# irfanfadhullah/unet_zoo

Measured on AMD Instinct MI355X. Metric: images/sec (fwd+bwd) at B=16 3x256x256, 1/2/4/8 MI355X, higher is better.
Workload: dtype bf16; 1 GPU; unet train step (zero_grad+fwd+BCE+bwd+clip+AdamW), B=16/GPU 3x256x256, random-init weights; global_batch=16, parallelism=dp1

## Files before the change

### include/unetzoo_hip.h

```cpp
#ifndef UNETZOO_HIP_H
#define UNETZOO_HIP_H

#include <stddef.h>
#include <stdint.h>

#ifdef __cplusplus
extern "C" {
#endif

#define UZ_ABI_VERSION 1

enum { UZ_F32 = 0, UZ_BF16 = 1 };

enum {
  UZ_OK = 0,
  UZ_EINVAL = -1,
  UZ_ENOTIMPL = -2
};

enum {
  UZ_TAPS_CONV = 0,
  UZ_TAPS_GATHER2X2 = 1,
  UZ_TAPS_CONV_UP2 = 2,
  UZ_TAPS_CONV_S2 = 3
};
enum {
  UZ_STORE_PLAIN = 0,
  UZ_STORE_SHUFFLE2X2 = 1
};

int uz_abi_version(void);
const char* uz_last_error_string(void);
int uz_profile_arm(void* start_event, void* stop_event);
int uz_profile_disarm(void);
int uz_build_ablate(void);
const char* uz_source_hash(void);
int uz_clock_probe(int iters, void* out_pairs, int workgroups, void* stream);
int uz_set_cu_reserve(int n);
int uz_get_cu_reserve(void);

typedef struct uz_conv_desc {
  int dtype;
  int N, H, W;
  int Hin, Win;
  int Cin, ldx;
  int Nout, ldy;
  int ntaps, taps_mode, dil;
  int store_mode, Co;
  int Hout, Wout;
} uz_conv_desc;

int uz_conv_igemm_grid_m(const uz_conv_desc* d);
int uz_conv_igemm_kernel_name(const uz_conv_desc* d, int with_workspace, char* buf, int cap);
int uz_conv_igemm(const uz_conv_desc* d, const void* x, const void* w_packed, const float* bias,
                  void* y, float* stats_partial, void* stream);
int uz_conv_igemm_res(const uz_conv_desc* d, const void* x, const void* w_packed, const float* bias,
                      const void* res, int ldres, void* y, void* stream);
int uz_conv_igemm_res_ws(const uz_conv_desc* d, const void* x, const void* w_packed, const float* bias,
                         const void* res, int ldres, void* y, void* workspace, void* stream);
long long uz_conv_igemm_workspace_bytes(const uz_conv_desc* d);
int uz_conv_igemm_ws_grid_m(const uz_conv_desc* d);
int uz_conv_igemm_ws(const uz_conv_desc* d, const void* x, const void* w_packed, const float* bias,
                     void* y, float* stats_partial, void* workspace, void* stream);
int uz_conv_igemm_bnred_supported(const uz_conv_desc* d);
int uz_conv_igemm_bnred(const uz_conv_desc* d, const void* x, const void* w_packed, void* y, const void* bn_y,
                        int ld_bny, const float* scale, const float* shift, const float* mean, const float* invstd,
                        float* partial, void* stream);

int uz_conv_igemm_xf_supported(const uz_conv_desc* d);
int uz_conv_igemm_xf(const uz_conv_desc* d, const void* x, const float* in_scale, const float* in_shift,
                     const void* w_packed, const float* bias, void* y, float* stats_partial, void* stream);

int uz_conv_igemm_bnact_supported(const uz_conv_desc* d);
int uz_conv_igemm_bnact(const uz_conv_desc* d, const void* x, const void* w_packed, const float* bias,
                        const float* out_scale, const float* out_shift, int relu, void* y, void* stream);

typedef struct uz_wgrad_desc {
  int dtype;
  int N, H, W;
  int Hr, Wr;
  int Ci, ldl;
  int Cj, ldr;
  int ntaps, taps_mode, dil;
} uz_wgrad_desc;

int uz_wgrad_split(const uz_wgrad_desc* d);
long long uz_wgrad_workspace_bytes(const uz_wgrad_desc* d);
int uz_wgrad(const uz_wgrad_desc* d, const void* L, const void* R, float* out, void* workspace,
             void* stream);
int uz_wgrad_kernel_name(const uz_wgrad_desc* d, char* buf, int cap);
int uz_wgrad_xf_supported(const uz_wgrad_desc* d);
int uz_wgrad_xf(const uz_wgrad_desc* d, const void* L, const void* R, const float* r_scale, const float* r_shift,
// ... 416 lines not shown
```

### unet_zoo_amd/_lib.py

```python
from __future__ import annotations

import ctypes
import os
from ctypes import POINTER, Structure, c_char_p, c_double, c_float, c_int, c_void_p

import torch

UZ_F32, UZ_BF16 = 0, 1
TAPS_CONV, TAPS_GATHER2X2, TAPS_CONV_UP2, TAPS_CONV_S2 = 0, 1, 2, 3
STORE_PLAIN, STORE_SHUFFLE2X2 = 0, 1
PACK_CONV_FWD, PACK_CONV_DGRAD, PACK_CONVT_FWD, PACK_CONVT_DGRAD, PACK_IM2COL, PACK_VEC_REPEAT = range(6)

LIB_NAME = "libunetzoo_hip.so"
LIB_PATH = os.environ.get("UNET_ZOO_AMD_LIB") or os.path.join(os.path.dirname(os.path.abspath(__file__)), LIB_NAME)

EXPORTS = (
    "uz_abi_version", "uz_last_error_string", "uz_build_ablate", "uz_source_hash", "uz_set_cu_reserve", "uz_get_cu_reserve", "uz_clock_probe", "uz_conv_igemm_grid_m", "uz_conv_igemm",
    "uz_wgrad_split", "uz_wgrad_workspace_bytes", "uz_wgrad", "uz_wgrad_kernel_name", "uz_wgrad_phase", "uz_wgrad_xf_supported", "uz_wgrad_xf", "uz_conv3x3_first_supported", "uz_conv3x3_first_rows", "uz_conv3x3_first_fwd",
    "uz_conv3x3_first_wgrad_workspace_bytes", "uz_conv3x3_first_wgrad", "uz_conv3x3_first_wgrad_bn", "uz_pack_weights", "uz_pack_weights_batched", "uz_pack_conv3x3_batched", "uz_im2col3x3_nchw", "uz_bn_finalize",
    "uz_bn_eval_scale", "uz_bn_relu_apply", "uz_bn_relu_bwd_workspace_bytes", "uz_bn_relu_bwd_reduce", "uz_bn_relu_bwd_apply",
    "uz_outconv_fwd", "uz_outconv_fwd_xf", "uz_outconv_bwd_workspace_bytes", "uz_outconv_bwd", "uz_outconv_bwd_rows", "uz_outconv_bwd_bnred", "uz_bn_relu_bwd_apply_head_supported", "uz_bn_relu_bwd_apply_head",
    "uz_colsum",
    "uz_attn_grid", "uz_attn_psi_fwd", "uz_attn_gate_fwd", "uz_attn_bwd_psi", "uz_attn_bwd_reduce",
    "uz_attn_bwd_apply", "uz_sum_rows", "uz_sum_rows_f32", "uz_sum2x2",
    "uz_bn_relu_add_apply", "uz_bn_relu_add_apply_fin", "uz_bn_relu_bwd_reduce_rows", "uz_bn_relu_bwd_apply_fin", "uz_bilinear_fwd", "uz_bilinear_bwd", "uz_resize_bilinear_fwd", "uz_resize_bilinear_bwd", "uz_resample2",
    "uz_pool_grad_combine",
    "uz_sideconv3x3_fwd", "uz_sideconv3x3_bwd_workspace_bytes", "uz_sideconv3x3_bwd",
    "uz_fuse1x1_fwd", "uz_fuse1x1_bwd_workspace_bytes", "uz_fuse1x1_bwd",
    "uz_conv_igemm_workspace_bytes", "uz_conv_igemm_ws_grid_m", "uz_conv_igemm_ws",
    "uz_conv_igemm_bnred_supported", "uz_conv_igemm_bnred", "uz_conv_igemm_xf_supported", "uz_conv_igemm_xf", "uz_conv_igemm_kernel_name", "uz_bn_bwd_finalize", "uz_profile_arm", "uz_profile_disarm",
    "uz_patchify", "uz_layernorm_fwd", "uz_layernorm_bwd_rows", "uz_layernorm_bwd", "uz_layernorm_act_bwd",
    "uz_ln_head_fwd", "uz_ln_head_bwd_workspace_bytes", "uz_ln_head_bwd", "uz_sum_rows_f32_ld",
    "uz_winattn_fwd", "uz_winattn_bwd_rows", "uz_winattn_bwd",
    "uz_colsum_workspace_bytes", "uz_colsum_ws", "uz_colstats_rows", "uz_colstats", "uz_cpb_fwd", "uz_cpb_bwd",
    "uz_cpb_fwd_batched", "uz_cpb_bwd_batched_workspace_bytes", "uz_cpb_bwd_batched",
    "uz_clip_adamw_workspace_bytes", "uz_clip_adamw",
    "uz_gelu_fwd", "uz_gelu_bwd", "uz_dwconv3x3", "uz_dwconv3x3_wgrad_rows", "uz_dwconv3x3_wgrad",
    "uz_space_to_depth", "uz_space_to_depth_crop", "uz_im2col_nchw", "uz_sra_fwd", "uz_sra_bwd_workspace_bytes", "uz_sra_bwd",
    "uz_bce_dice_workspace_bytes", "uz_bce_dice", "uz_colsum_batched_workspace_bytes", "uz_colsum_batched", "uz_sum_rows_f32_batched", "uz_conv_igemm_res", "uz_wgrad_multi_workspace_bytes", "uz_wgrad_multi", "uz_conv_igemm_res_ws",
    "uz_add_relu", "uz_relu_bwd", "uz_pil_resample_h_u8", "uz_pil_resample_v_f32",
    "uz_gemm_nt", "uz_softmax_fwd", "uz_softmax_bwd", "uz_adaptive_avgpool_fwd", "uz_adaptive_avgpool_bwd",
    "uz_rowdot_f32", "uz_cast_rows", "uz_wgrad_batched_workspace_bytes", "uz_wgrad_batched", "uz_wgrad_batched2",
    "uz_softmax_workspace_bytes", "uz_add_map", "uz_dropout", "uz_chanscale_relu", "uz_chanattn_probs_fwd", "uz_chanattn_probs_bwd",
    "uz_conv5x5_grid_m", "uz_conv5x5", "uz_wgrad5x5_workspace_bytes", "uz_wgrad5x5",
    "uz_bn_elu_apply", "uz_bn_elu_bwd_rows", "uz_bn_elu_bwd_reduce", "uz_bn_elu_bwd_apply",
    "uz_conv_igemm_bnact_supported", "uz_conv_igemm_bnact", "uz_conv3x3_first_fwd_bnact",
    "uz_region_loss_workspace_bytes", "uz_region_loss",
    "uz_class_loss_workspace_bytes", "uz_class_loss",
)


class ConvDesc(Structure):
    _fields_ = [(n, c_int) for n in (
        "dtype", "N", "H", "W", "Hin", "Win", "Cin", "ldx", "Nout", "ldy", "ntaps", "taps_mode",
        "dil", "store_mode", "Co", "Hout", "Wout")]


class WgradDesc(Structure):
    _fields_ = [(n, c_int) for n in (
        "dtype", "N", "H", "W", "Hr", "Wr", "Ci", "ldl", "Cj", "ldr", "ntaps", "taps_mode", "dil")]


class Conv5Desc(Structure):
    _fields_ = [(n, c_int) for n in ("dtype", "N", "H", "W", "Cin", "ldx", "Nout", "ldy", "ksize")]


class Wgrad5Desc(Structure):
    _fields_ = [(n, c_int) for n in ("dtype", "N", "H", "W", "Ci", "ldl", "Cj", "ldr", "ksize", "CiOut", "CjOut")]


# ... 62 lines not shown
REGION_MAX_ITEMS = 64


class RegionItem(Structure):
    _fields_ = [("logits", c_void_p), ("target", c_void_p), ("dlogits", c_void_p), ("weight", c_float)]


class RegionDesc(Structure):
    _fields_ = [("n_items", c_int), ("n", ctypes.c_longlong), ("groups", c_int)] \
        + [(n, c_float) for n in ("w_bce", "w_region", "alpha", "beta", "smooth", "gamma", "pos_weight")] \
        + [("metric_item", c_int)]


CLASS_MAX_ITEMS = 16
CLASS_MAX_K = 32
CLASS_REDUCE_BATCH, CLASS_REDUCE_IMAGE = 0, 1


class ClassItem(Structure):
    _fields_ = [("logits", c_void_p), ("dlogits", c_void_p), ("weight", c_float)]


class ClassDesc(Structure):
    _fields_ = [("n_items", c_int), ("N", c_int), ("K", c_int), ("HW", ctypes.c_longlong)] \
        + [(n, c_float) for n in ("w_ce", "w_dice", "smooth", "label_smoothing")] \
        + [(n, c_int) for n in ("ignore_index", "reduce", "include_background", "square", "metric_item")]


class HipLibraryError(RuntimeError):
    pass


_lib = None


def load():
    global _lib
    if _lib is not None:
        return _lib
    if not os.path.exists(LIB_PATH):
        raise HipLibraryError(
            f"{LIB_PATH} not found: the HIP kernel library is not built. Run "
            "`python -c 'import __graft_entry__ as g; g.build()'` from the repo root. "
            "unet_zoo_amd has no CPU fallback.")
    lib = ctypes.CDLL(LIB_PATH)
    lib.uz_abi_version.restype = c_int
    lib.uz_last_error_string.restype = c_char_p
    lib.uz_source_hash.restype = c_char_p
    lib.uz_source_hash.argtypes = []
    vp, ip, fp = c_void_p, c_int, c_float
    lib.uz_set_cu_reserve.argtypes = [c_int]
    lib.uz_clock_probe.argtypes = [c_int, vp, c_int, vp]
    lib.uz_get_cu_reserve.argtypes = []
    lib.uz_conv_igemm_grid_m.argtypes = [POINTER(ConvDesc)]
    lib.uz_conv_igemm.argtypes = [POINTER(ConvDesc), vp, vp, vp, vp, vp, vp]
    lib.uz_conv_igemm_res.argtypes = [POINTER(ConvDesc), vp, vp, vp, vp, ip, vp, vp]
    lib.uz_conv_igemm_res_ws.argtypes = [POINTER(ConvDesc), vp, vp, vp, vp, ip, vp, vp, vp]
    lib.uz_conv_igemm_workspace_bytes.argtypes = [POINTER(ConvDesc)]
    lib.uz_conv_igemm_ws_grid_m.argtypes = [POINTER(ConvDesc)]
    lib.uz_conv_igemm_ws.argtypes = [POINTER(ConvDesc), vp, vp, vp, vp, vp, vp, vp]
    lib.uz_conv_igemm_bnred_supported.argtypes = [POINTER(ConvDesc)]
    lib.uz_conv_igemm_xf_supported.argtypes = [POINTER(ConvDesc)]
    lib.uz_conv_igemm_xf.argtypes = [POINTER(ConvDesc), vp, vp, vp, vp, vp, vp, vp, vp]
    lib.uz_conv_igemm_bnact_supported.argtypes = [POINTER(ConvDesc)]
    lib.uz_conv_igemm_bnact.argtypes = [POINTER(ConvDesc), vp, vp, vp, vp, vp, c_int, vp, vp]
    lib.uz_conv_igemm_kernel_name.argtypes = [POINTER(ConvDesc), c_int, c_char_p, c_int]
    lib.uz_profile_arm.argtypes = [vp, vp]
    lib.uz_profile_disarm.argtypes = []
    lib.uz_conv_igemm_bnred.argtypes = [POINTER(ConvDesc), vp, vp, vp, vp, c_int, vp, vp, vp, vp, vp, vp]
    lib.uz_bn_bwd_finalize.argtypes = [vp, c_int, c_int, vp, vp, vp, vp]
    lib.uz_patchify.argtypes = [ip, vp, ip, ip, ip, ip, ip, ip, vp, vp]
    lib.uz_layernorm_fwd.argtypes = [POINTER(LnDesc), vp, vp, vp, vp, vp, vp, vp, vp]
    lib.uz_layernorm_act_bwd.argtypes = [POINTER(LnDesc), vp, vp, vp, vp, vp, vp, vp, vp]
    lib.uz_layernorm_bwd_rows.argtypes = [POINTER(LnDesc)]
    lib.uz_layernorm_bwd.argtypes = [POINTER(LnDesc), vp, vp, vp, vp, vp, vp, vp, vp]
    lib.uz_ln_head_fwd.argtypes = [POINTER(LnDesc), vp, vp, vp, vp, vp, ip, vp, vp, vp]
    lib.uz_ln_head_bwd_workspace_bytes.argtypes = [POINTER(LnDesc), ip]
    lib.uz_ln_head_bwd.argtypes = [POINTER(LnDesc), vp, vp, vp, vp, ip, vp, vp, vp, vp, vp, vp, vp, vp, vp]
    lib.uz_sum_rows_f32_ld.argtypes = [vp, ip, ip, ip, vp, ip, vp, vp]
    lib.uz_winattn_fwd.argtypes = [POINTER(WinAttnDesc), vp, vp, vp, vp, vp, vp]
    lib.uz_winattn_bwd_rows.argtypes = [POINTER(WinAttnDesc)]
    lib.uz_winattn_bwd.argtypes = [POINTER(WinAttnDesc), vp, vp, vp, vp, vp, vp, ip, vp, ip, vp, vp]
    lib.uz_colstats_rows.argtypes = [ip, ip, ip]
    lib.uz_colstats.argtypes = [ip, vp, ip, ip, ip, vp, vp]
    lib.uz_cpb_fwd.argtypes = [vp, vp, vp, vp, vp, ip, ip, ip, vp, vp]
    lib.uz_cpb_bwd.argtypes = [vp, vp, vp, vp, vp, ip, ip, ip, vp, vp, vp, vp, vp]
    lib.uz_cpb_fwd_batched.argtypes = [vp, ip, vp]
    lib.uz_cpb_bwd_batched_workspace_bytes.argtypes = [vp, ip]
    lib.uz_cpb_bwd_batched.argtypes = [vp, ip, vp, vp]
    lib.uz_clip_adamw_workspace_bytes.argtypes = []
    lib.uz_clip_adamw.argtypes = [vp, vp, vp, vp, ctypes.c_longlong, fp, fp, fp, fp, fp, fp, vp, vp, vp]
    lib.uz_wgrad_split.argtypes = [POINTER(WgradDesc)]
    lib.uz_wgrad_workspace_bytes.argtypes = [POINTER(WgradDesc)]
    lib.uz_wgrad.argtypes = [POINTER(WgradDesc), vp, vp, vp, vp, vp]
    lib.uz_wgrad_kernel_name.argtypes = [POINTER(WgradDesc), c_char_p, c_int]
    lib.uz_wgrad_phase.argtypes = [POINTER(WgradDesc), vp, vp, vp, vp, vp, c_int]
    lib.uz_wgrad_xf_supported.argtypes = [POINTER(WgradDesc)]
    lib.uz_wgrad_xf.argtypes = [POINTER(WgradDesc), vp, vp, vp, vp, vp, vp, vp, c_int]
    lib.uz_conv3x3_first_supported.argtypes = [ip, ip, ip]
    lib.uz_conv3x3_first_rows.argtypes = [ip, ip, ip]
    lib.uz_conv3x3_first_fwd.argtypes = [ip, vp, ip, ip, ip, ip, vp, vp, ip, vp, ip, vp, vp]
    lib.uz_conv3x3_first_fwd_bnact.argtypes = [ip, vp, ip, ip, ip, ip, vp, vp, ip, vp, vp, ip, vp, ip, vp]
    lib.uz_conv3x3_first_wgrad_workspace_bytes.argtypes = [ip, ip, ip, ip]
    lib.uz_conv3x3_first_wgrad_workspace_bytes.restype = ctypes.c_longlong
    lib.uz_conv3x3_first_wgrad.argtypes = [ip, vp, ip, ip, ip, ip, vp, ip, ip, vp, vp, vp]
    lib.uz_conv3x3_first_wgrad_bn.argtypes = [ip, vp, ip, ip, ip, ip, vp, ip, vp, ip, vp, vp, vp, vp, vp, ctypes.c_double, ip, vp, vp, vp]
# ... 105 lines not shown
        if name not in ("uz_last_error_string", "uz_source_hash"):
            fn.restype = ctypes.c_longlong if name.endswith("_workspace_bytes") else c_int
    if lib.uz_abi_version() != 1:
        raise HipLibraryError("libunetzoo_hip.so ABI version mismatch; rebuild it")
    _lib = lib
    return lib


def _fail(rc: int, what: str):
    msg = load().uz_last_error_string().decode("utf-8", "replace")
    raise HipLibraryError(f"{what} failed (code {rc}): {msg}")


def check(rc: int, what: str) -> None:
    if rc != 0:
        _fail(rc, what)


def check_count(rc: int, what: str) -> int:
    if rc < 0:
        _fail(rc, what)
    return rc


def region_loss_workspace_bytes(desc: "RegionDesc") -> int:
    return check_count(load().uz_region_loss_workspace_bytes(ctypes.byref(desc)), "uz_region_loss_workspace_bytes")


def region_loss(desc: "RegionDesc", items, out2: torch.Tensor, workspace: torch.Tensor) -> None:
    check(load().uz_region_loss(ctypes.byref(desc), items, out2.data_ptr(), workspace.data_ptr(), stream_ptr()),
          "uz_region_loss")


def class_loss_workspace_bytes(desc: "ClassDesc") -> int:
    return check_count(load().uz_class_loss_workspace_bytes(ctypes.byref(desc)), "uz_class_loss_workspace_bytes")


def class_loss(desc: "ClassDesc", items, labels: torch.Tensor, class_weight, out2: torch.Tensor, counts: torch.Tensor,
               workspace: torch.Tensor) -> None:
    check(load().uz_class_loss(ctypes.byref(desc), items, labels.data_ptr(),
                               class_weight.data_ptr() if class_weight is not None else None, out2.data_ptr(),
                               counts.data_ptr() if counts is not None else None, workspace.data_ptr(), stream_ptr()),
          "uz_class_loss")


def set_cu_reserve(n: int) -> None:
    check(load().uz_set_cu_reserve(int(n)), "uz_set_cu_reserve")


def get_cu_reserve() -> int:
    return int(load().uz_get_cu_reserve())


def mfma_clock_ghz(settle_s: float = 0.6, iters: int = 40000) -> dict:
    import time
    lib = load()
    dev = torch.device("cuda", torch.cuda.current_device())
    out = torch.zeros(256, 2, dtype=torch.int64, device=dev)
    torch.cuda.synchronize()
    t_end = time.perf_counter() + settle_s
    while time.perf_counter() < t_end:
        for _ in range(4):
            check(lib.uz_clock_probe(iters, out.data_ptr(), 256, stream_ptr()), "uz_clock_probe")
        torch.cuda.synchronize()
    e0, e1 = torch.cuda.Event(enable_timing=True), torch.cuda.Event(enable_timing=True)
    e0.record()
    check(lib.uz_clock_probe(iters, out.data_ptr(), 256, stream_ptr()), "uz_clock_probe")
    e1.record()
    torch.cuda.synchronize()
    o = out.double().cpu()
    ghz = (o[:, 0] / o[:, 1] / 10.0)
    flops = 256.0 * 8 * iters * 8 * 2.0 * 16 * 16 * 32
    return {"median_ghz": round(float(ghz.median()), 4), "min_ghz": round(float(ghz.min()), 4),
            "max_ghz": round(float(ghz.max()), 4),
            "probe_tflops": round(flops / (e0.elapsed_time(e1) * 1e-3) / 1e12, 1)}


def stream_ptr() -> int:
    return torch.cuda.current_stream().cuda_stream


def dtype_code(dt: torch.dtype) -> int:
    if dt == torch.float32:
        return UZ_F32
    if dt == torch.bfloat16:
        return UZ_BF16
    raise ValueError(f"unsupported run dtype {dt}; use torch.float32 or torch.bfloat16")


def require_cuda(*tensors: torch.Tensor) -> None:
    for t in tensors:
        if t is not None and not t.is_cuda:
            raise HipLibraryError(
                "unet_zoo_amd kernels run on an MI355X only: got a CPU tensor. Move the model and "
                "inputs to 'cuda' (there is no CPU fallback in the product path).")
```

### unet_zoo_amd/csrc/uz_common.h

```cpp
#pragma once
#include <hip/hip_runtime.h>
#include <stdarg.h>
#include <stdint.h>
#include <stdio.h>
#include "../../include/unetzoo_hip.h"

typedef __bf16 bf16_t;
typedef __attribute__((ext_vector_type(16))) float f32x16;
typedef __attribute__((ext_vector_type(4))) float f32x4;
typedef __attribute__((ext_vector_type(8))) __bf16 bf16x8;
typedef __attribute__((ext_vector_type(4))) __bf16 bf16x4;

#include <hip/hip_ext.h>
bool uz_prof_take(hipEvent_t* e0, hipEvent_t* e1);
#undef hipLaunchKernelGGL
#define hipLaunchKernelGGL(kern, grid, block, shm, stream, ...)                                              \
  do {                                                                                                       \
    hipEvent_t uz_e0_, uz_e1_;                                                                               \
    if (uz_prof_take(&uz_e0_, &uz_e1_))                                                                      \
      hipExtLaunchKernelGGL(kern, dim3(grid), dim3(block), (shm), (stream), uz_e0_, uz_e1_, 0, __VA_ARGS__);   \
    else                                                                                                     \
      kern<<<dim3(grid), dim3(block), (shm), (stream)>>>(__VA_ARGS__);                                       \
  } while (0)

// ... 130 lines not shown
  const float *scale, *shift;
};
struct UzBnAct {
  const float *scale, *shift;
  int relu;
};
int uz_direct_launch(const uz_conv_desc* d, const UzDirectPlan& p, const void* x, const void* w,
                     const float* bias, void* y, float* stats, hipStream_t s, const UzBnRed* br = nullptr,
                     float* part = nullptr,
                     const UzXf* xf = nullptr, const UzBnAct* ba = nullptr);

enum { UZ_PP_512 = 0,
       UZ_PP_512X64 = 1,
       UZ_PP_256 = 2,
       UZ_PP_256W16 = 3,
       UZ_PP_128W16 = 4 };
struct UzPpPlan {
  int cfg, bn, th_n, tw_n, ntiles, tiles_n, grid_m;
  int ksplit, cps;
};
int uz_pp_plan(const uz_conv_desc* d, UzPpPlan* p);
int uz_pp_launch(const uz_conv_desc* d, const UzPpPlan& p, const void* x, const void* w, const float* bias, void* y,
                 float* stats, hipStream_t s, const UzBnRed* br = nullptr, float* part = nullptr, const UzXf* xf = nullptr,
                 const UzBnAct* ba = nullptr);
int uz_pp_xf_channels(const UzPpPlan& p);

struct UzWgrad2Plan {
  int big, one_tap, gather, kw, kr, tiles_i, tiles_j, kg, units, upb, split, nslabs, H, W;
  int wide9;
  int v9, bi;
};
int uz_wgrad9_plan(const uz_wgrad_desc* d, UzWgrad2Plan* p);
int uz_wgrad9_launch(const uz_wgrad_desc* d, const UzWgrad2Plan& p, const void* L, const void* R, float* slab, hipStream_t s,
                     const UzXf* xf = nullptr);
const char* uz_wgrad9_name(const UzWgrad2Plan& p);
int uz_wgrad_g4_plan(const uz_wgrad_desc* d, UzWgrad2Plan* p);
int uz_wgrad_g4_launch(const uz_wgrad_desc* d, const UzWgrad2Plan& p, const void* L, const void* R, float* slab, hipStream_t s);
int uz_wgrad3x3_plan(const uz_wgrad_desc* d, UzWgrad2Plan* p, int batch = 1);
int uz_wgrad3x3_launch(const uz_wgrad_desc* d, const UzWgrad2Plan& p, const void* L, const void* R,
                       float* slab, hipStream_t s, int batch = 1, long long lb_bytes = 0, long long rb_bytes = 0,
                       long long slab_stride = 0,
                       int batch2 = 1, long long lb2_bytes = 0, long long rb2_bytes = 0,
                       const UzXf* xf = nullptr);

struct UzWgradMultiItem {
  const uz_wgrad_desc* d;
  UzWgrad2Plan p;
  const void *L, *R;
  float* slab;
};
int uz_wgrad3x3_multi_max();
int uz_wgrad3x3_multi_launch(const UzWgradMultiItem* items, int n, hipStream_t s);

struct UzGemmPlan {
  int bn, bm, nst, tiles_m, tiles_n, grid_m;
  int ksplit, cps;
};
int uz_gemm_dma_plan(const uz_conv_desc* d, UzGemmPlan* p);
long long uz_gemm_dma_workspace_bytes(const uz_conv_desc* d);
int uz_gemm_dma_launch(const uz_conv_desc* d, const UzGemmPlan& p, const void* x, const void* w,
                       const float* bias, void* y, float* stats, hipStream_t s, const void* res = nullptr,
                       int ldres = 0, const UzBnRed* br = nullptr, float* part = nullptr);
```

### unet_zoo_amd/csrc/uz_igemm.hip

```cpp
#include "uz_common.h"
#include <string.h>

namespace {

struct IgemmArgs {
  const void* x;
  const void* w;
  void* y;
  const float* bias;
  float* stats;
  int M, H, W, Hin, Win, Cin, ldx, Nout, ldy, K, ntaps, mode, dil, store, Co, tiles_m, Hout, Wout;
  float* part;
  int tpg;
  const float* act_scale;
  const float* act_shift;
  int act_relu;
};

template <typename T> struct Mma;
template <> struct Mma<bf16_t> {
  static __device__ __forceinline__ void run(const Vec16<bf16_t>& a, const Vec16<bf16_t>& b,
                                             f32x16& c) {
    c = __builtin_amdgcn_mfma_f32_32x32x16_bf16(*reinterpret_cast<const bf16x8*>(&a),
                                                *reinterpret_cast<const bf16x8*>(&b), c, 0, 0, 0);
// ... 403 lines not shown
  if (cap < 1) cap = 1;
  p->grid_m = p->tiles_m < cap ? p->tiles_m : cap;
  p->split = 1;
  const int vec_ = d->dtype == UZ_BF16 ? 8 : 4;
  if (d->taps_mode == UZ_TAPS_CONV && d->ntaps == 9 && d->store_mode == UZ_STORE_PLAIN &&
      p->tiles_m * p->tiles_n <= UZ_NUM_CU / 2 && d->Nout % vec_ == 0 && d->ldy % vec_ == 0 &&
      !(uz_tune_flags() & 8)) {
    p->split = 9;
    reduce_geometry(M, d->Nout, vec_, p);
  }
  return UZ_OK;
}

template <typename T>
int launch(const uz_conv_desc* d, const Plan& p, const IgemmArgs& a, hipStream_t s) {
  dim3 grid(p.grid_m, p.tiles_n, a.part != nullptr ? p.split : 1), block(256);
  if (a.act_scale != nullptr) {
    if (p.bn == 64) hipLaunchKernelGGL((igemm_kernel<T, 128, 64, 2, 2, true>), grid, block, 0, s, a);
    else hipLaunchKernelGGL((igemm_kernel<T, 128, 128, 2, 2, true>), grid, block, 0, s, a);
    UZ_LAUNCH_CHECK("uz_conv_igemm_bnact");
    return UZ_OK;
  }
  if (p.bn == 64) {
    hipLaunchKernelGGL((igemm_kernel<T, 128, 64, 2, 2>), grid, block, 0, s, a);
  } else {
    hipLaunchKernelGGL((igemm_kernel<T, 128, 128, 2, 2>), grid, block, 0, s, a);
  }
  UZ_LAUNCH_CHECK("uz_conv_igemm");
  if (a.part != nullptr) {
    constexpr int VEC = ElemTraits<T>::VEC;
    const size_t shm = (size_t)256 * 2 * VEC * sizeof(float);
    hipLaunchKernelGGL((igemm_split_reduce_kernel<T>), dim3(p.rgx, p.rgy), dim3(p.rbx, p.rby), shm, s,
                       static_cast<const float*>(a.part), p.split, a.M, a.Nout, a.bias, static_cast<T*>(a.y), a.ldy, a.stats,
                       static_cast<const T*>(nullptr), 0);
    UZ_LAUNCH_CHECK("uz_conv_igemm(split reduce)");
  }
  return UZ_OK;
}

bool generic_path(const uz_conv_desc* d) {
  UzDirectPlan dp;
  UzGemmPlan gp;
  return !uz_direct_plan(d, &dp) && !uz_gemm_dma_plan(d, &gp);
}

}

extern "C" int uz_conv_igemm_grid_m(const uz_conv_desc* d) {
  Plan p;
  const int rc = make_plan(d, &p);
  if (rc != UZ_OK) return rc;
  UzDirectPlan dp;
  if (uz_direct_plan(d, &dp)) return dp.grid_m;
  UzGemmPlan gp;
  if (uz_gemm_dma_plan(d, &gp)) return gp.grid_m;
  return p.grid_m;
}

extern "C" int uz_conv_igemm_kernel_name(const uz_conv_desc* d, int with_workspace, char* buf, int cap) {
  Plan p;
  const int rc = make_plan(d, &p);
  if (rc != UZ_OK) return rc;
  UZ_REQUIRE(buf != nullptr && cap > 0, "uz_conv_igemm_kernel_name: no buffer");
  const char* dt = d->dtype == UZ_BF16 ? "bf16" : "f32";
  char name[96];
  UzDirectPlan dp;
  UzGemmPlan gp;
  if (uz_direct_plan(d, &dp)) {
    const char* up = d->taps_mode == UZ_TAPS_CONV_UP2 ? "_up2" : "";
    static const char* const ppn[8] = {"pp512", "pp512x64", "pp256", "pp256w16", "pp128w16", "?", "?", "?"};
    if (dp.bres == 3) snprintf(name, sizeof(name), "conv3x3_%s_%s%s%s", ppn[dp.ppcfg & 7], dt, up, (dp.ksplit > 1 && with_workspace) ? "_splitk" : "");
    else if (dp.bres == 2) snprintf(name, sizeof(name), "conv3x3_res64_%s%s", dt, up);
    else snprintf(name, sizeof(name), "conv3x3_direct_%s_bn%d%s%s", dt, dp.bn, dp.bres == 1 ? "_resident" : "", up);
  } else if (uz_gemm_dma_plan(d, &gp)) {
    snprintf(name, sizeof(name), "gemm_dma_%s", dt);
  } else {
    snprintf(name, sizeof(name), "igemm_%s_128x%d%s", dt, p.bn, (p.split > 1 && with_workspace) ? "_tapsplit" : "");
  }
  const int len = (int)strlen(name);
  snprintf(buf, (size_t)cap, "%s", name);
  return len;
}

extern "C" long long uz_conv_igemm_workspace_bytes(const uz_conv_desc* d) {
  Plan p;
  const int rc = make_plan(d, &p);
  if (rc != UZ_OK) return rc;
  {
    UzDirectPlan dp;
    if (uz_direct_plan(d, &dp) && dp.bres == 3 && dp.ksplit > 1)
      return (long long)dp.ksplit * d->N * d->H * d->W * d->Nout * (long long)sizeof(float);
  }
  {
    UzDirectPlan dp;
    const long long gb = uz_direct_plan(d, &dp) ? 0 : uz_gemm_dma_workspace_bytes(d);
    if (gb > 0) return gb;
  }
  if (p.split <= 1 || !generic_path(d)) return 0;
  return (long long)p.split * d->N * d->H * d->W * d->Nout * (long long)sizeof(float);
}

extern "C" int uz_conv_igemm_ws_grid_m(const uz_conv_desc* d) {
  Plan p;
  const int rc = make_plan(d, &p);
  if (rc != UZ_OK) return rc;
  {
    UzDirectPlan dp;
    if (uz_direct_plan(d, &dp) && dp.bres == 3 && dp.ksplit > 1) {
      Plan rp;
      reduce_geometry((long long)d->N * d->H * d->W, d->Nout, 8, &rp);
      return rp.rgx;
    }
  }
  {
    UzDirectPlan dp;
    if (!uz_direct_plan(d, &dp) && uz_gemm_dma_workspace_bytes(d) > 0) {
      Plan rp;
      reduce_geometry((long long)d->N * d->H * d->W, d->Nout, 8, &rp);
      return rp.rgx;
    }
  }
  if (p.split > 1 && generic_path(d)) return p.rgx;
  return uz_conv_igemm_grid_m(d);
}

extern "C" int uz_conv_igemm(const uz_conv_desc* d, const void* x, const void* w_packed,
// ... 48 lines not shown
  if (!uz_direct_plan(d, &dp) || dp.bres != 3 || dp.ksplit > 1) return 0;
  UzPpPlan pp = {dp.ppcfg, dp.bn, dp.th_n, dp.tw_n, dp.ntiles, dp.tiles_n, dp.grid_m, dp.ksplit, dp.cps};
  return d->Cin <= uz_pp_xf_channels(pp) ? 1 : 0;
}

extern "C" int uz_conv_igemm_xf(const uz_conv_desc* d, const void* x, const float* in_scale, const float* in_shift,
                                const void* w_packed, const float* bias, void* y, float* stats_partial, void* stream) {
  Plan p;
  const int rc = make_plan(d, &p);
  if (rc != UZ_OK) return rc;
  UZ_REQUIRE(x && w_packed && y && in_scale && in_shift, "uz_conv_igemm_xf: null pointer");
  UZ_REQUIRE(((uintptr_t)x & 15) == 0 && ((uintptr_t)w_packed & 15) == 0 && ((uintptr_t)y & 15) == 0,
             "uz_conv_igemm_xf: x / w / y must be 16-byte aligned");
  if (!uz_conv_igemm_xf_supported(d)) {
    uz_set_error("uz_conv_igemm_xf: only bf16 3x3 problems of the ping-pong configurations whose LDS image leaves room for "
                 "the channel table (ask uz_conv_igemm_xf_supported)");
    return UZ_ENOTIMPL;
  }
  UzDirectPlan dp;
  UZ_REQUIRE(uz_direct_plan(d, &dp), "uz_conv_igemm_xf: no plan");
  const UzXf xf = {in_scale, in_shift};
  return uz_direct_launch(d, dp, x, w_packed, bias, y, stats_partial, static_cast<hipStream_t>(stream), nullptr, nullptr, &xf);
}

extern "C" int uz_conv_igemm_bnred_supported(const uz_conv_desc* d) {
  UzDirectPlan dp;
  UzGemmPlan gp;
  if (d == nullptr || d->dtype != UZ_BF16) return 0;
  if (uz_direct_plan(d, &dp)) return dp.bres != 2 ? 1 : 0;
  return (d->store_mode == UZ_STORE_PLAIN && uz_gemm_dma_plan(d, &gp)) ? 1 : 0;
}

extern "C" int uz_conv_igemm_bnred(const uz_conv_desc* d, const void* x, const void* w_packed, void* y,
                                   const void* bn_y, int ld_bny, const float* scale, const float* shift,
                                   const float* mean, const float* invstd, float* partial, void* stream) {
  Plan p;
  const int rc = make_plan(d, &p);
  if (rc != UZ_OK) return rc;
  UZ_REQUIRE(x && w_packed && y && bn_y && scale && shift && mean && invstd && partial,
             "uz_conv_igemm_bnred: null pointer");
  UZ_REQUIRE(((uintptr_t)x & 15) == 0 && ((uintptr_t)w_packed & 15) == 0 && ((uintptr_t)y & 15) == 0 &&
                 ((uintptr_t)bn_y & 15) == 0, "uz_conv_igemm_bnred: x / w / y / bn_y must be 16-byte aligned");
  UZ_REQUIRE(ld_bny >= d->Nout && ld_bny % 8 == 0, "uz_conv_igemm_bnred: bad ld_bny %d", ld_bny);
  UzDirectPlan dp;
  UzGemmPlan gp;
  if (!uz_conv_igemm_bnred_supported(d)) {
    uz_set_error("uz_conv_igemm_bnred: only bf16 problems of the direct 3x3 kernels with the LDS-staged epilogue and of "
                 "the LDS-DMA GEMM with a plain store (ask uz_conv_igemm_bnred_supported)");
    return UZ_ENOTIMPL;
  }
  const UzBnRed br = {bn_y, ld_bny, scale, shift, mean, invstd};
  if (uz_direct_plan(d, &dp))
    return uz_direct_launch(d, dp, x, w_packed, nullptr, y, partial, static_cast<hipStream_t>(stream), &br);
  UZ_REQUIRE(uz_gemm_dma_plan(d, &gp), "uz_conv_igemm_bnred: no plan");
  return uz_gemm_dma_launch(d, gp, x, w_packed, nullptr, y, partial, static_cast<hipStream_t>(stream), nullptr, 0, &br);
}

extern "C" int uz_conv_igemm_ws(const uz_conv_desc* d, const void* x, const void* w_packed,
                                const float* bias, void* y, float* stats_partial, void* workspace,
                                void* stream) {
  Plan p;
  const int rc = make_plan(d, &p);
  if (rc != UZ_OK) return rc;
  UZ_REQUIRE(x && w_packed && y, "uz_conv_igemm: null pointer");
  UZ_REQUIRE(((uintptr_t)x & 15) == 0 && ((uintptr_t)w_packed & 15) == 0 && ((uintptr_t)y & 15) == 0,
             "uz_conv_igemm: x / w / y must be 16-byte aligned");
  UzDirectPlan dp;
  if (uz_direct_plan(d, &dp)) {
    if (dp.bres == 3 && dp.ksplit > 1 && workspace != nullptr) {
      hipStream_t s = static_cast<hipStream_t>(stream);
      const int r1 = uz_direct_launch(d, dp, x, w_packed, nullptr, y, nullptr, s, nullptr, static_cast<float*>(workspace));
      if (r1 != UZ_OK) return r1;
      Plan rp;
      const long long M = (long long)d->N * d->H * d->W;
      reduce_geometry(M, d->Nout, 8, &rp);
      const size_t shm = (size_t)256 * 2 * 8 * sizeof(float);
      hipLaunchKernelGGL((igemm_split_reduce_kernel<bf16_t>), dim3(rp.rgx, rp.rgy), dim3(rp.rbx, rp.rby), shm, s,
                         static_cast<const float*>(workspace), dp.ksplit, (int)M, d->Nout, bias, static_cast<bf16_t*>(y), d->ldy,
                         stats_partial, static_cast<const bf16_t*>(nullptr), 0);
      UZ_LAUNCH_CHECK("uz_conv_igemm(split-K reduce)");
      return UZ_OK;
    }
    return uz_direct_launch(d, dp, x, w_packed, bias, y, stats_partial, static_cast<hipStream_t>(stream));
  }
  UzGemmPlan gp;
  if (uz_gemm_dma_plan(d, &gp)) {
    if (gp.ksplit > 1 && workspace != nullptr)
      return gemm_split_k(d, gp, x, w_packed, bias, nullptr, 0, y, workspace, static_cast<hipStream_t>(stream), stats_partial);
    return uz_gemm_dma_launch(d, gp, x, w_packed, bias, y, stats_partial, static_cast<hipStream_t>(stream));
  }
  IgemmArgs a;
  a.x = x;
  a.w = w_packed;
  a.y = y;
  a.bias = bias;
  a.stats = stats_partial;
  a.M = d->N * d->H * d->W;
  a.H = d->H;
  a.W = d->W;
  a.Hin = d->Hin;
  a.Win = d->Win;
  a.Cin = d->Cin;
  a.ldx = d->ldx;
  a.Nout = d->Nout;
  a.ldy = d->ldy;
  a.K = d->ntaps * d->Cin;
  a.ntaps = d->ntaps;
  a.mode = d->taps_mode;
  a.dil = d->dil;
  a.store = d->store_mode;
  a.Co = d->Co;
  a.Hout = d->Hout ? d->Hout : 2 * d->H;
  a.Wout = d->Wout ? d->Wout : 2 * d->W;
  a.tiles_m = p.tiles_m;
  a.part = (p.split > 1 && workspace != nullptr) ? static_cast<float*>(workspace) : nullptr;
  a.tpg = (d->ntaps + p.split - 1) / p.split;
  a.act_scale = nullptr;
  a.act_shift = nullptr;
  a.act_relu = 0;
  hipStream_t s = static_cast<hipStream_t>(stream);
  return d->dtype == UZ_BF16 ? launch<bf16_t>(d, p, a, s) : launch<float>(d, p, a, s);
}

extern "C" int uz_conv_igemm_bnact_supported(const uz_conv_desc* d) {
  Plan p;
  if (d == nullptr || make_plan(d, &p) != UZ_OK) return 0;
  if (d->store_mode != UZ_STORE_PLAIN || !(d->taps_mode == UZ_TAPS_CONV || d->taps_mode == UZ_TAPS_CONV_UP2)) return 0;
  UzDirectPlan dp;
  UzGemmPlan gp;
  if (uz_direct_plan(d, &dp)) {
    if (dp.bres == 2) return 0;
    if (dp.bres == 3 && dp.ksplit > 1) return 0;
    return 1;
  }
  if (uz_gemm_dma_plan(d, &gp)) return 0;
  return p.split > 1 ? 0 : 1;
}
// ... 51 lines not shown
```

Measured before the change: 2563 images/sec.

## Add persistent double-buffered LDS-DMA GEMM for transposed-conv and 2x2 gather shapes

Adds a new persistent GEMM kernel with one workgroup per CU. It keeps the weight tile resident in LDS and double-buffers activation tiles through buffer-load-to-LDS, so the load of the next tile overlaps the MFMA work on the current one. The kernel is routed ahead of the existing LDS-DMA GEMM for two shapes: the 1x1 up-conv with shuffle store (Cin 128, Nout 256) and the 2x2 gather (Cin 64, Nout 128), with an optional fused BN-backward reduction. It aims to cut per-tile launch and weight reload costs and to hide load latency, at the cost of large LDS use (one block per CU) and a runtime mask to disable it.

```diff
diff --git a/include/unetzoo_hip.h b/include/unetzoo_hip.h
--- a/include/unetzoo_hip.h
+++ b/include/unetzoo_hip.h
@@ -38,6 +38,8 @@
 int uz_clock_probe(int iters, void* out_pairs, int workgroups, void* stream);
 int uz_set_cu_reserve(int n);
 int uz_get_cu_reserve(void);
+int uz_set_gemm_pp(int forward, int gather);
+int uz_get_gemm_pp(void);
 
 typedef struct uz_conv_desc {
   int dtype;
diff --git a/unet_zoo_amd/_lib.py b/unet_zoo_amd/_lib.py
--- a/unet_zoo_amd/_lib.py
+++ b/unet_zoo_amd/_lib.py
@@ -15,7 +15,7 @@
 LIB_PATH = os.environ.get("UNET_ZOO_AMD_LIB") or os.path.join(os.path.dirname(os.path.abspath(__file__)), LIB_NAME)
 
 EXPORTS = (
-    "uz_abi_version", "uz_last_error_string", "uz_build_ablate", "uz_source_hash", "uz_set_cu_reserve", "uz_get_cu_reserve", "uz_clock_probe", "uz_conv_igemm_grid_m", "uz_conv_igemm",
+    "uz_abi_version", "uz_last_error_string", "uz_build_ablate", "uz_source_hash", "uz_set_cu_reserve", "uz_get_cu_reserve", "uz_set_gemm_pp", "uz_get_gemm_pp", "uz_clock_probe", "uz_conv_igemm_grid_m", "uz_conv_igemm",
     "uz_wgrad_split", "uz_wgrad_workspace_bytes", "uz_wgrad", "uz_wgrad_kernel_name", "uz_wgrad_phase", "uz_wgrad_xf_supported", "uz_wgrad_xf", "uz_conv3x3_first_supported", "uz_conv3x3_first_rows", "uz_conv3x3_first_fwd",
     "uz_conv3x3_first_wgrad_workspace_bytes", "uz_conv3x3_first_wgrad", "uz_conv3x3_first_wgrad_bn", "uz_pack_weights", "uz_pack_weights_batched", "uz_pack_conv3x3_batched", "uz_im2col3x3_nchw", "uz_bn_finalize",
     "uz_bn_eval_scale", "uz_bn_relu_apply", "uz_bn_relu_bwd_workspace_bytes", "uz_bn_relu_bwd_reduce", "uz_bn_relu_bwd_apply",
@@ -184,6 +184,8 @@
     lib.uz_set_cu_reserve.argtypes = [c_int]
     lib.uz_clock_probe.argtypes = [c_int, vp, c_int, vp]
     lib.uz_get_cu_reserve.argtypes = []
+    lib.uz_set_gemm_pp.argtypes = [c_int, c_int]
+    lib.uz_get_gemm_pp.argtypes = []
     lib.uz_conv_igemm_grid_m.argtypes = [POINTER(ConvDesc)]
     lib.uz_conv_igemm.argtypes = [POINTER(ConvDesc), vp, vp, vp, vp, vp, vp]
     lib.uz_conv_igemm_res.argtypes = [POINTER(ConvDesc), vp, vp, vp, vp, ip, vp, vp]
@@ -395,6 +397,15 @@
     return int(load().uz_get_cu_reserve())
 
 
+def set_gemm_pp(forward: bool = True, gather: bool = True) -> None:
+    check(load().uz_set_gemm_pp(int(bool(forward)), int(bool(gather))), "uz_set_gemm_pp")
+
+
+def get_gemm_pp() -> tuple:
+    m = int(load().uz_get_gemm_pp())
+    return bool(m & 1), bool(m & 2)
+
+
 def mfma_clock_ghz(settle_s: float = 0.6, iters: int = 40000) -> dict:
     import time
     lib = load()
diff --git a/unet_zoo_amd/csrc/uz_common.h b/unet_zoo_amd/csrc/uz_common.h
--- a/unet_zoo_amd/csrc/uz_common.h
+++ b/unet_zoo_amd/csrc/uz_common.h
@@ -206,6 +206,15 @@
 int uz_wgrad3x3_multi_max();
 int uz_wgrad3x3_multi_launch(const UzWgradMultiItem* items, int n, hipStream_t s);
 
+enum { UZ_GPP_FWD_128X256 = 0,
+       UZ_GPP_GATHER_64X128 = 1 };
+struct UzGemmPpPlan {
+  int cfg, bm, sub, tiles_m, grid_m;
+};
+int uz_gemm_pp_plan(const uz_conv_desc* d, UzGemmPpPlan* p);
+int uz_gemm_pp_launch(const uz_conv_desc* d, const UzGemmPpPlan& p, const void* x, const void* w, const float* bias, void* y,
+                      float* stats, hipStream_t s, const UzBnRed* br = nullptr);
+
 struct UzGemmPlan {
   int bn, bm, nst, tiles_m, tiles_n, grid_m;
   int ksplit, cps;
diff --git a/unet_zoo_amd/csrc/uz_gemm_pp.hip b/unet_zoo_amd/csrc/uz_gemm_pp.hip
--- /dev/null
+++ b/unet_zoo_amd/csrc/uz_gemm_pp.hip
@@ -0,0 +1,381 @@
+#include <atomic>
+#include "uz_common.h"
+
+namespace {
+
+struct PArgs {
+  const void* x;
+  const void* w;
+  void* y;
+  const float* bias;
+  float* stats;
+  const void* bn_y;
+  const float *bn_scale, *bn_shift, *bn_mean, *bn_invstd;
+  int ld_bny;
+  unsigned xbytes, wbytes;
+  int M, H, W, Hin, Win, Cin, ldx, Nout, ldy, K, Co, Hout, Wout, tiles_m;
+};
+
+typedef __attribute__((address_space(3))) void* lds_ptr_t;
+typedef __attribute__((address_space(3))) char* lds_char_ptr;
+typedef unsigned u32x2 __attribute__((ext_vector_type(2)));
+
+template <int N> __device__ __forceinline__ void wait_vmcnt() {
+  static_assert(N >= 0 && N <= 63, "vmcnt range");
+  asm volatile("s_waitcnt vmcnt(%0)" ::"n"(N) : "memory");
+}
+__device__ __forceinline__ void wait_lgkm0() { asm volatile("s_waitcnt lgkmcnt(0)" ::: "memory"); }
+template <int OFF> __device__ __forceinline__ void lds_read16(f32x4& dst, unsigned lds_addr) {
+  static_assert(OFF >= 0 && OFF < 65536, "ds offset");
+  asm volatile("ds_read_b128 %0, %1 offset:%2" : "=v"(dst) : "v"(lds_addr), "n"(OFF));
+}
+__device__ __forceinline__ void lds_write8(unsigned lds_addr, const u32x2& v) {
+  asm volatile("ds_write_b64 %0, %1" ::"v"(lds_addr), "v"(v) : "memory");
+}
+__device__ __forceinline__ void pin16(f32x4& v) { asm volatile("" : "+v"(v)); }
+template <int V> struct IntC { static constexpr int value = V; };
+template <int K, int NK> struct Steps {
+  template <typename F> static __device__ __forceinline__ void run(F& f) {
+    f(IntC<K>());
+    Steps<K + 1, NK>::run(f);
+  }
+};
+template <int NK> struct Steps<NK, NK> {
+  template <typename F> static __device__ __forceinline__ void run(F&) {}
+};
+
+template <int BM, int BN, int NSLAB, int SUB, bool GATHER, bool BNRED>
+__global__ __launch_bounds__(512, 1) void gemm_pp_kernel(const PArgs a) {
+  typedef bf16_t T;
+  constexpr int ES = 2, VEC = 8;
+  constexpr int WM = 2, WN = 4, TM = BM / (32 * WM), TN = BN / (32 * WN);
+  constexpr int A_TILE = BM * NSLAB * 128, B_BYTES = BN * NSLAB * 128;
+  constexpr int RSB = BN * ES;
+  constexpr int STG_BYTES = WM * 32 * RSB;
+  constexpr int OFF_B = 2 * A_TILE, OFF_STG = OFF_B + B_BYTES;
+  constexpr int NAPW = A_TILE / 1024 / 8, NBPW = B_BYTES / 1024 / 8;
+  constexpr int PPS_A = BM / 8, PPS_B = BN / 8;
+  constexpr int NK = NSLAB * 4;
+  constexpr int CPR = BN * ES / 16, RPP = 512 / CPR, NPASS = WM * 32 / RPP;
+  constexpr int NSTORE = TM * NPASS;
+  static_assert(TM >= 1 && TM <= 2 && TN >= 1 && TN <= 2 && A_TILE % 8192 == 0 && B_BYTES % 8192 == 0, "tile");
+  static_assert(OFF_STG + STG_BYTES <= 160 * 1024 && CPR % 8 == 0 && RPP % 8 == 0 && 512 * 2 * VEC * 4 <= OFF_B, "LDS");
+  static_assert(!BNRED || TM == 1, "the fused sums keep one round of pre-activation values in registers");
+  __shared__ __attribute__((aligned(1024))) char smem[OFF_STG + STG_BYTES];
+
+  const int tid = threadIdx.x, lane = tid & 63;
+  const int wave = __builtin_amdgcn_readfirstlane(tid >> 6);
+  const int wm = wave / WN, wn = wave % WN;
+  const int l31 = lane & 31, lh = lane >> 5;
+  const unsigned smem_u = (unsigned)(size_t)(lds_char_ptr)smem;
+  const __amdgpu_buffer_rsrc_t xr = __builtin_amdgcn_make_buffer_rsrc(const_cast<void*>(a.x), 0, a.xbytes, 0x00020000);
+  const __amdgpu_buffer_rsrc_t wr = __builtin_amdgcn_make_buffer_rsrc(const_cast<void*>(a.w), 0, a.wbytes, 0x00020000);
+  T* __restrict__ yg = static_cast<T*>(a.y);
+  const int HW = a.H * a.W;
+
+  unsigned a_rd[4], b_rd[4];
+#pragma unroll
+  for (int q = 0; q < 4; ++q) {
+    const unsigned co = (unsigned)(((2 * q + lh) ^ ((l31 >> 1) & 7)) << 4);
+    a_rd[q] = smem_u + (unsigned)((wm * TM * 32 + l31) * 128) + co;
+    b_rd[q] = smem_u + (unsigned)(OFF_B + (wn * TN * 32 + l31) * 128) + co;
+  }
+  const unsigned stg_w = smem_u + (unsigned)(OFF_STG + (wm * 32 + l31) * RSB + 8 * lh);
+  const int rrow = tid / CPR, cc = tid % CPR;
+  const unsigned stg_r = smem_u + (unsigned)(OFF_STG + rrow * RSB + ((cc ^ (rrow & 7)) << 4));
+  const int nthr = cc * VEC;
+  const int abt = GATHER ? 0 : nthr / a.Co;
+  const int cot = GATHER ? nthr : nthr - abt * a.Co;
+
+  float bq[TN][16];
+  if constexpr (!BNRED) {
+    const float* bp = a.bias != nullptr ? a.bias : static_cast<const float*>(a.w);
+    f32x4 bl[TN][4];
+#pragma unroll
+    for (int j = 0; j < TN; ++j)
+#pragma unroll
+      for (int q = 0; q < 4; ++q) bl[j][q] = *reinterpret_cast<const f32x4*>(bp + wn * TN * 32 + j * 32 + 8 * q + 4 * lh);
+#pragma unroll
+    for (int j = 0; j < TN; ++j)
+#pragma unroll
+      for (int q = 0; q < 4; ++q) pin16(bl[j][q]);
+#pragma unroll
+    for (int j = 0; j < TN; ++j)
+#pragma unroll
+      for (int r = 0; r < 16; ++r) bq[j][r] = a.bias != nullptr ? bl[j][r >> 2][r & 3] : 0.f;
+  }
+  float bsc[VEC], bsh[VEC];
+  if constexpr (BNRED) {
+#pragma unroll
+    for (int e = 0; e < VEC; e += 4) {
+      *reinterpret_cast<f32x4*>(&bsc[e]) = *reinterpret_cast<const f32x4*>(a.bn_scale + nthr + e);
+      *reinterpret_cast<f32x4*>(&bsh[e]) = *reinterpret_cast<const f32x4*>(a.bn_shift + nthr + e);
+    }
+  }
+  float sq1[VEC], sq2[VEC];
+#pragma unroll
+  for (int e = 0; e < VEC; ++e) sq1[e] = sq2[e] = 0.f;
+
+  auto issue_a = [&](int tile, int buf) {
+    const int m0t = tile * BM;
+    const int ncb = a.Cin >> 6;
+#pragma unroll
+    for (int k = 0; k < NAPW; ++k) {
+      const int pc = wave + 8 * k;
+      const int s = pc / PPS_A;
+      const int row = (pc % PPS_A) * 8 + (lane >> 3);
+      const int m = m0t + row;
+      const unsigned coff = (unsigned)(((lane & 7) ^ ((row >> 1) & 7)) << 4);
+      unsigned pix, cb;
+      if constexpr (GATHER) {
+        const int tap = s / ncb;
+        cb = (unsigned)(s - tap * ncb);
+        const int img = m / HW, rem = m - img * HW;
+        const int h = rem / a.W, w = rem - h * a.W;
+        pix = (unsigned)((img * a.Hin + 2 * h + (tap >> 1)) * a.Win + 2 * w + (tap & 1));
+      } else {
+        pix = (unsigned)m;
+        cb = (unsigned)s;
+      }
+      const unsigned off = pix * (unsigned)(a.ldx * ES) + cb * 128u + coff;
+      __builtin_amdgcn_raw_ptr_buffer_load_lds(xr, (lds_ptr_t)(smem + buf * A_TILE + pc * 1024), 16, off, 0, 0, 0);
+    }
+  };
+
+  const int nit = ((a.tiles_m / SUB - (int)blockIdx.x + (int)gridDim.x - 1) / (int)gridDim.x) * SUB;
+  auto tile_of = [&](int it) { return ((int)blockIdx.x + (it / SUB) * (int)gridDim.x) * SUB + it % SUB; };
+  if (nit > 0) {
+#pragma unroll
+    for (int k = 0; k < NBPW; ++k) {
+      const int pc = wave + 8 * k;
+      const int s = pc / PPS_B;
+      const int n = (pc % PPS_B) * 8 + (lane >> 3);
+      const unsigned off = (unsigned)n * (unsigned)(a.K * ES) + (unsigned)(s * 128) + (unsigned)(((lane & 7) ^ ((n >> 1) & 7)) << 4);
+      __builtin_amdgcn_raw_ptr_buffer_load_lds(wr, (lds_ptr_t)(smem + OFF_B + pc * 1024), 16, off, 0, 0, 0);
+    }
+    issue_a(tile_of(0), 0);
+  }
+
+  int buf = 0;
+  for (int it = 0; it < nit; ++it) {
+    const int m0 = tile_of(it) * BM;
+    if (it == 0) wait_vmcnt<0>();
+    else wait_vmcnt<NSTORE>();
+    __builtin_amdgcn_s_barrier();
+
+    long long orow[TM][NPASS];
+#pragma unroll
+    for (int i = 0; i < TM; ++i)
+#pragma unroll
+      for (int k = 0; k < NPASS; ++k) {
+        const int rr = rrow + k * RPP;
+        const int m = m0 + (rr >> 5) * (32 * TM) + i * 32 + (rr & 31);
+        if constexpr (GATHER) {
+          orow[i][k] = m;
+        } else {
+          const int img = m / HW, rem = m - img * HW;
+          const int h = rem / a.W, w = rem - h * a.W;
+          orow[i][k] = ((long long)img * a.Hout + 2 * h + (abt >> 1)) * a.Wout + 2 * w + (abt & 1);
+        }
+      }
+    Vec16<T> yb[NPASS];
+    if constexpr (BNRED) {
+      const T* by = static_cast<const T*>(a.bn_y);
+#pragma unroll
+      for (int k = 0; k < NPASS; ++k) yb[k] = ld16(by + (size_t)orow[0][k] * a.ld_bny + nthr);
+    }
+    {
+      if (it + 1 < nit) issue_a(tile_of(it + 1), buf ^ 1);
+    }
+
+    f32x16 acc[TM][TN];
+#pragma unroll
+    for (int i = 0; i < TM; ++i)
+#pragma unroll
+      for (int j = 0; j < TN; ++j)
+#pragma unroll
+        for (int r = 0; r < 16; ++r) acc[i][j][r] = 0.f;
+
+    f32x4 fa[2][TM], fb[2][TN];
+    const unsigned abuf = (unsigned)(buf * A_TILE);
+    auto rd = [&](auto kc) __attribute__((always_inline)) {
+      constexpr int k = decltype(kc)::value, s = k >> 2, q = k & 3, set = k & 1;
+      lds_read16<s * BM * 128>(fa[set][0], a_rd[q] + abuf);
+      if constexpr (TM > 1) lds_read16<s * BM * 128 + 4096>(fa[set][TM - 1], a_rd[q] + abuf);
+      lds_read16<s * BN * 128>(fb[set][0], b_rd[q]);
+      if constexpr (TN > 1) lds_read16<s * BN * 128 + 4096>(fb[set][TN - 1], b_rd[q]);
+    };
+    auto step = [&](auto kc) __attribute__((always_inline)) {
+      constexpr int k = decltype(kc)::value, set = k & 1;
+      wait_lgkm0();
+#pragma unroll
+      for (int i = 0; i < TM; ++i) pin16(fa[set][i]);
+#pragma unroll
+      for (int j = 0; j < TN; ++j) pin16(fb[set][j]);
+      if constexpr (k + 1 < NK) rd(IntC<k + 1>());
+#pragma unroll
+      for (int i = 0; i < TM; ++i)
+#pragma unroll
+        for (int j = 0; j < TN; ++j)
+          acc[i][j] = __builtin_amdgcn_mfma_f32_32x32x16_bf16(*reinterpret_cast<const bf16x8*>(&fb[set][j]),
+                                                              *reinterpret_cast<const bf16x8*>(&fa[set][i]), acc[i][j], 0, 0, 0);
+    };
+    rd(IntC<0>());
+    Steps<0, NK>::run(step);
+
+    if constexpr (BNRED) {
+#pragma unroll
+      for (int k = 0; k < NPASS; ++k) pin16(*reinterpret_cast<f32x4*>(&yb[k]));
+    }
+#pragma unroll
+    for (int i = 0; i < TM; ++i) {
+      if (i > 0) __builtin_amdgcn_s_barrier();
+#pragma unroll
+      for (int j = 0; j < TN; ++j)
+#pragma unroll
+        for (int q = 0; q < 4; ++q) {
+          bf16x4 pk;
+#pragma unroll
+          for (int e = 0; e < 4; ++e) pk[e] = (bf16_t)(BNRED ? acc[i][j][4 * q + e] : acc[i][j][4 * q + e] + bq[j][4 * q + e]);
+          const int c = wn * (TN * 4) + j * 4 + q;
+          lds_write8(stg_w + (unsigned)((c ^ (l31 & 7)) << 4), __builtin_bit_cast(u32x2, pk));
+        }
+      wait_lgkm0();
+      __builtin_amdgcn_s_barrier();
+      f32x4 vr[NPASS];
+#pragma unroll
+      for (int k = 0; k < NPASS; ++k) lds_read16<0>(vr[k], stg_r + (unsigned)(k * RPP * RSB));
+      wait_lgkm0();
+#pragma unroll
+      for (int k = 0; k < NPASS; ++k) pin16(vr[k]);
+#pragma unroll
+      for (int k = 0; k < NPASS; ++k) {
+        const Vec16<T> vb = __builtin_bit_cast(Vec16<T>, vr[k]);
+        st16(yg + (size_t)orow[i][k] * a.ldy + cot, vb);
+        if constexpr (BNRED) {
+#pragma unroll
+          for (int e = 0; e < VEC; ++e) {
+            const float yv = (float)yb[k].v[e];
+            const float dz = fmaf(yv, bsc[e], bsh[e]) > 0.f ? (float)vb.v[e] : 0.f;
+            sq1[e] += dz;
+            sq2[e] += dz * yv;
+          }
+        } else {
+#pragma unroll
+          for (int e = 0; e < VEC; ++e) {
+            const float fv = (float)vb.v[e];
+            sq1[e] += fv;
+            sq2[e] += fv * fv;
+          }
+        }
+      }
+    }
+    buf ^= 1;
+  }
+
+  if (a.stats != nullptr) {
+    wait_vmcnt<0>();
+    __syncthreads();
+    float* red = reinterpret_cast<float*>(smem);
+#pragma unroll
+    for (int e = 0; e < VEC; ++e) {
+      red[tid * 2 * VEC + e] = sq1[e];
+      red[tid * 2 * VEC + VEC + e] = sq2[e];
+    }
+    __syncthreads();
+    if (tid < 2 * BN) {
+      const int which = tid / BN, ch = tid - which * BN;
+      const int c8 = ch / VEC, e = ch - c8 * VEC;
+      float t = 0.f;
+      for (int k = c8; k < 512; k += CPR) t += red[k * 2 * VEC + which * VEC + e];
+      if constexpr (BNRED) {
+        if (which == 1) {
+          float t0 = 0.f;
+          for (int k = c8; k < 512; k += CPR) t0 += red[k * 2 * VEC + e];
+          t = a.bn_invstd[ch] * (t - a.bn_mean[ch] * t0);
+        }
+      }
+      a.stats[((size_t)blockIdx.x * 2 + which) * a.Nout + ch] = t;
+    }
+  }
+}
+
+std::atomic<int> g_pp_mask{3};
+
+}
+
+extern "C" int uz_set_gemm_pp(int forward, int gather) {
+  g_pp_mask.store((forward ? 1 : 0) | (gather ? 2 : 0), std::memory_order_relaxed);
+  return UZ_OK;
+}
+extern "C" int uz_get_gemm_pp(void) { return g_pp_mask.load(std::memory_order_relaxed); }
+
+int uz_gemm_pp_plan(const uz_conv_desc* d, UzGemmPpPlan* p) {
+  if (d->dtype != UZ_BF16) return 0;
+  const int mask = g_pp_mask.load(std::memory_order_relaxed);
+  const bool fwd = d->taps_mode == UZ_TAPS_CONV && d->ntaps == 1 && d->store_mode == UZ_STORE_SHUFFLE2X2 && d->Co % 64 == 0;
+  const bool gath = d->taps_mode == UZ_TAPS_GATHER2X2 && d->ntaps == 4 && d->store_mode == UZ_STORE_PLAIN;
+  if (!(fwd && (mask & 1)) && !(gath && (mask & 2))) return 0;
+  if (d->Cin % 64 != 0 || d->ldx % 8 != 0 || d->ldy % 8 != 0) return 0;
+  const long long pin = (long long)d->N * d->Hin * d->Win;
+  const long long xbytes = (pin - 1) * d->ldx * 2 + (long long)d->Cin * 2;
+  const long long wbytes = (long long)d->Nout * d->ntaps * d->Cin * 2;
+  if (xbytes >= (1LL << 31) || wbytes >= (1LL << 31)) return 0;
+  const long long M = (long long)d->N * d->H * d->W;
+  if (fwd && d->Nout == 256 && d->Cin == 128) {
+    p->cfg = UZ_GPP_FWD_128X256;
+    p->bm = 128;
+    p->sub = 1;
+  } else if (gath && d->Nout == 128 && d->Cin == 64) {
+    p->cfg = UZ_GPP_GATHER_64X128;
+    p->bm = 64;
+    p->sub = 4;
+    if (((M + 255) / 256) * 2 <= UZ_NUM_CU) return 0;
+  } else {
+    return 0;
+  }
+  if (M % (p->bm * p->sub) != 0) return 0;
+  p->tiles_m = (int)(M / p->bm);
+  const int runs = p->tiles_m / p->sub, cap = UZ_NUM_CU;
+  p->grid_m = runs < cap ? runs : cap;
+  return 1;
+}
+
+int uz_gemm_pp_launch(const uz_conv_desc* d, const UzGemmPpPlan& p, const void* x, const void* w, const float* bias, void* y,
+                      float* stats, hipStream_t s, const UzBnRed* br) {
+  PArgs a;
+  a.x = x;
+  a.w = w;
+  a.y = y;
+  a.bias = bias;
+  a.stats = stats;
+  a.bn_y = br ? br->y : nullptr;
+  a.bn_scale = br ? br->scale : nullptr;
+  a.bn_shift = br ? br->shift : nullptr;
+  a.bn_mean = br ? br->mean : nullptr;
+  a.bn_invstd = br ? br->invstd : nullptr;
+  a.ld_bny = br ? br->ldy : 0;
+  if (br) UZ_REQUIRE(p.cfg == UZ_GPP_GATHER_64X128 && stats != nullptr, "uz_conv_igemm_bnred(gemm_dma_pp): gather form with partial rows");
+  a.xbytes = (unsigned)(((long long)d->N * d->Hin * d->Win - 1) * d->ldx * 2 + (long long)d->Cin * 2);
+  a.wbytes = (unsigned)((long long)d->Nout * d->ntaps * d->Cin * 2);
+  a.M = d->N * d->H * d->W;
+  a.H = d->H;
+  a.W = d->W;
+  a.Hin = d->Hin;
+  a.Win = d->Win;
+  a.Hout = d->Hout ? d->Hout : 2 * d->H;
+  a.Wout = d->Wout ? d->Wout : 2 * d->W;
+  a.Cin = d->Cin;
+  a.ldx = d->ldx;
+  a.Nout = d->Nout;
+  a.ldy = d->ldy;
+  a.K = d->ntaps * d->Cin;
+  a.Co = d->Co > 0 ? d->Co : d->Nout;
+  a.tiles_m = p.tiles_m;
+  dim3 grid(p.grid_m), block(512);
+  if (p.cfg == UZ_GPP_FWD_128X256) hipLaunchKernelGGL((gemm_pp_kernel<128, 256, 2, 1, false, false>), grid, block, 0, s, a);
+  else if (br) hipLaunchKernelGGL((gemm_pp_kernel<64, 128, 4, 4, true, true>), grid, block, 0, s, a);
+  else hipLaunchKernelGGL((gemm_pp_kernel<64, 128, 4, 4, true, false>), grid, block, 0, s, a);
+  UZ_LAUNCH_CHECK("uz_conv_igemm(gemm_dma_pp)");
+  return UZ_OK;
+}
diff --git a/unet_zoo_amd/csrc/uz_igemm.hip b/unet_zoo_amd/csrc/uz_igemm.hip
--- a/unet_zoo_amd/csrc/uz_igemm.hip
+++ b/unet_zoo_amd/csrc/uz_igemm.hip
@@ -479,6 +479,8 @@
   if (rc != UZ_OK) return rc;
   UzDirectPlan dp;
   if (uz_direct_plan(d, &dp)) return dp.grid_m;
+  UzGemmPpPlan pp;
+  if (uz_gemm_pp_plan(d, &pp)) return pp.grid_m;
   UzGemmPlan gp;
   if (uz_gemm_dma_plan(d, &gp)) return gp.grid_m;
   return p.grid_m;
@@ -499,6 +501,8 @@
     if (dp.bres == 3) snprintf(name, sizeof(name), "conv3x3_%s_%s%s%s", ppn[dp.ppcfg & 7], dt, up, (dp.ksplit > 1 && with_workspace) ? "_splitk" : "");
     else if (dp.bres == 2) snprintf(name, sizeof(name), "conv3x3_res64_%s%s", dt, up);
     else snprintf(name, sizeof(name), "conv3x3_direct_%s_bn%d%s%s", dt, dp.bn, dp.bres == 1 ? "_resident" : "", up);
+  } else if (UzGemmPpPlan pp; uz_gemm_pp_plan(d, &pp)) {
+    snprintf(name, sizeof(name), "gemm_dma_pp_%s", dt);
   } else if (uz_gemm_dma_plan(d, &gp)) {
     snprintf(name, sizeof(name), "gemm_dma_%s", dt);
   } else {
@@ -653,6 +657,9 @@
   const UzBnRed br = {bn_y, ld_bny, scale, shift, mean, invstd};
   if (uz_direct_plan(d, &dp))
     return uz_direct_launch(d, dp, x, w_packed, nullptr, y, partial, static_cast<hipStream_t>(stream), &br);
+  UzGemmPpPlan pp;
+  if (uz_gemm_pp_plan(d, &pp))
+    return uz_gemm_pp_launch(d, pp, x, w_packed, nullptr, y, partial, static_cast<hipStream_t>(stream), &br);
   UZ_REQUIRE(uz_gemm_dma_plan(d, &gp), "uz_conv_igemm_bnred: no plan");
   return uz_gemm_dma_launch(d, gp, x, w_packed, nullptr, y, partial, static_cast<hipStream_t>(stream), nullptr, 0, &br);
 }
@@ -684,6 +691,9 @@
     }
     return uz_direct_launch(d, dp, x, w_packed, bias, y, stats_partial, static_cast<hipStream_t>(stream));
   }
+  UzGemmPpPlan pp;
+  if (uz_gemm_pp_plan(d, &pp))
+    return uz_gemm_pp_launch(d, pp, x, w_packed, bias, y, stats_partial, static_cast<hipStream_t>(stream));
   UzGemmPlan gp;
   if (uz_gemm_dma_plan(d, &gp)) {
     if (gp.ksplit > 1 && workspace != nullptr)
```

After: 2575 images/sec (median of 6 runs). About the same (+0.4%).
